# LayoutLLM-T2I/LayoutLLM-T2I

Hardware: AMD Instinct MI355X
Metric: 512x512 50-step images/sec (PLMS, CFG 7.5, layout-conditioned GLIGEN UNet) (higher is better)
Workload: dtype fp16 (fp32 accumulate); 1 GPU; configs[1]: 512x512, 50 PLMS steps, batch=4/GPU, 8 grounding boxes/image, fp16; survey_config=2, unet_forwards_per_image=102, parallelism=replicas x1, one weight broadcast, no per-step collectives

## Files before the change

layoutllm_t2i_amd/csrc/gemm8.hip:

```cpp
#include "common.h"
#include "gligen_hip.h"
#include "gemm_shared.h"
#include "opts.h"
#include <atomic>
#include <type_traits>

#ifndef G8_S3_PHASES
#define G8_S3_PHASES 3
#endif

namespace {

template <int BM_, int BN>
struct G8 {
    static constexpr int BM = BM_;
    static constexpr int NA = BM / 64;
    static constexpr int MI = BM / 64;
    static constexpr int MH = BM / 128;
    static constexpr int BK = 64;
    static constexpr int PW = BN / 2;
    static constexpr int TN = PW / 16;
    static constexpr int A_BYTES = BM * BK * 2;
    static constexpr int B_BYTES = BN * BK * 2;
    static constexpr int STAGE = A_BYTES + B_BYTES;
// ... 306 lines not shown
            }
        };
        constexpr int XA = 5;
        const half_t* xptr[XA];
        unsigned xrb = 0u;
#pragma unroll
        for (int u = 0; u < XA; ++u) {
            const int j = 8 * (u < 4 ? 4 * wave + u : 32) + srow;
            const int mc = m0 - 1 + j;
            xptr[u] = zsrc;
            if (mc >= 0 && mc < M) {
                int oy, ox;
                pix(mc, oy, ox);
                xrb |= ((oy >= 1 ? 1u : 0u) | 2u | (oy + 1 < cg.Hin ? 4u : 0u)) << (3 * u);
                xptr[u] = cg.in + (size_t)mc * cg.Cin + ((sslot ^ ((j >> 1) & 7)) << 3);
            }
        }
        const int xrow = 64 * wm + lr;
        auto xfrag = [&](const int j) __attribute__((always_inline)) -> int { return j * 128 + ((lq ^ ((j >> 1) & 7)) << 4); };
        const int xzero = X::A_BYTES + (lq << 4);
        const int xo1 = xfrag(xrow + 1);
        int xo0[MI], xo2[MI];
#pragma unroll
        for (int mi = 0; mi < MI; ++mi) {
            int oy, ox;
            pix(m0 + xrow + 16 * mi, oy, ox);
            xo0[mi] = ox == 0 ? xzero : xfrag(xrow + 16 * mi);
            xo2[mi] = ox == cg.Win - 1 ? xzero : xfrag(xrow + 16 * mi + 2);
        }
        const int xb_off = (PW * grp + lr) * 128 + fsw;
        if (tid < 16) *reinterpret_cast<uint4*>(smem + (tid >> 3) * X::A_STRIDE + X::A_BYTES + ((tid & 7) << 4)) = make_uint4(0u, 0u, 0u, 0u);
        asm volatile("s_waitcnt lgkmcnt(0)" ::: "memory");

        int xa_ky = 0, xa_cb = kt_begin / 9, xb_kt = kt_begin;
        int xa_off = -cg.Win * cg.Cin + (xa_cb << 6);
        int xa_rd = 0, xa_is = 0, xb_rd = 0, xb_is = 0;
        auto xa_advance = [&]() __attribute__((always_inline)) {
            if (++xa_ky == 3) { xa_ky = 0; ++xa_cb; }
            xa_off = (xa_ky - 1) * cg.Win * cg.Cin + (xa_cb << 6);
        };
        auto x_src = [&](const int id) __attribute__((always_inline)) -> const half_t* {
            const half_t* src;
            if (id < 8) {
                const uint64_t a = reinterpret_cast<uint64_t>(xptr[id < XA ? id : 0] + xa_off), z = reinterpret_cast<uint64_t>(zsrc);
                const uint64_t keep = (uint64_t)0 - (uint64_t)((xrb >> (3 * id + xa_ky)) & 1u);
                src = reinterpret_cast<const half_t*>((a & keep) | (z & ~keep));
                if constexpr (DBG & 2) src = zsrc;
            } else {
                const int j = id - 8 < C::NB0 ? id - 8 : 0;
                src = ((bmask >> j) & 1u) ? bptr[j] + (xb_kt << 6) : zsrc;
                if constexpr (DBG & 4) src = zsrc;
            }
            return src;
        };
        auto x_fire = [&](const int id, const half_t* src) __attribute__((always_inline)) {
            if (id < 8) glds16(src, reinterpret_cast<half_t*>(smem + xa_is * X::A_STRIDE + (id < 4 ? 4 * wave + id : 32) * 1024));
            else glds16(src, reinterpret_cast<half_t*>(smem + X::B_BASE + xb_is * X::B_BYTES + (bunit0 + id - 8) * 1024));
        };
        const bool has_a4 = wave == 4;
        const bool has_b2 = C::NB0 > 2 && nb > 2;

#pragma unroll
        for (int u = 0; u < 4; ++u) x_fire(u, x_src(u));
        if (has_a4) x_fire(4, x_src(4));
        xa_advance();
        xa_is = 1;
#pragma unroll
        for (int s = 0; s < 2; ++s) {
// ... 237 lines not shown
    } else {
        for (; t + 2 < nkt; ++t) ktile(std::true_type{});
        for (; t < nkt; ++t) ktile(std::false_type{});
    }
    if (grp == 0) G8_SBAR();
    if constexpr (DBG & 1) ts2 = __builtin_readcyclecounter();

    constexpr int EPS = PW + 4;
    constexpr int CG8 = PW / 8;
    constexpr int ITEMS = 32 * CG8;
    static_assert(ITEMS % 64 == 0, "whole sweeps");
    float* stage = reinterpret_cast<float*>(smem) + wave * (32 * EPS);
    const int epi = p.epi;
    const float* __restrict__ bias = p.bias;
    float gate = 1.0f;
    if (splitk == 1 && epi == GL_EPI_GATE_RES) gate = p.gate[0];
    const int nbase = n0 + PW * grp;
    half_t* outp = reinterpret_cast<half_t*>(p.out);
    constexpr int NQ = ITEMS / 64;
    const bool vt_wave = p.vt != nullptr && nbase >= p.vt_col0;
    const bool generic = splitk == 1 && !vt_wave && epi != GL_EPI_GEGLU;
    auto orow = [&](const int m) __attribute__((always_inline)) -> int {
        if constexpr (UPF) {
            const int hw = cg.Hin * cg.Win;
            const int b = m / hw;
            const int rr = m - b * hw;
            const int y = rr / cg.Win;
            const int x = rr - y * cg.Win;
            return (b * cg.Hout + 2 * y + py) * cg.Wout + 2 * x + px;
        } else {
            return m;
        }
    };
    Fin8Aux aux[MH][NQ];
    if (generic) {
#pragma unroll
        for (int h = 0; h < MH; ++h)
#pragma unroll
            for (int q = 0; q < NQ; ++q) {
                const int idx = lane + 64 * q;
                const int r = idx / CG8, c = (idx - r * CG8) * 8;
                const int m = m0 + (BM / 4) * wm + 32 * h + r, n = nbase + c;
                if (m < Mrows && n < N) fin8_load(p, orow(m), n, aux[h][q]);
            }
    }
    float vt_bias[2] = {0.0f, 0.0f};
    if (splitk == 1 && vt_wave && bias) {
#pragma unroll
        for (int j = 0; j < 2; ++j) {
            const int col = 64 * j + lane;
            if (col < PW && nbase + col < N) vt_bias[j] = bias[nbase + col];
        }
    }
    float gg_bias[16];
#pragma unroll
    for (int j = 0; j < 16; ++j) gg_bias[j] = 0.0f;
    if constexpr (PW == 64) {
        if (splitk == 1 && epi == GL_EPI_GEGLU && bias) {
            const int nx = nbase + (lane & 3) * 8;
            if (nx < N) {
#pragma unroll
                for (int j = 0; j < 8; ++j) { gg_bias[j] = bias[nx + j]; gg_bias[8 + j] = bias[nx + 32 + j]; }
            }
        }
    }
#pragma unroll
// ... 82 lines not shown
                        const float4 g0 = *reinterpret_cast<const float4*>(stage + r * EPS + pc + 32);
                        const float4 g1 = *reinterpret_cast<const float4*>(stage + r * EPS + pc + 36);
                        float xv[8] = {x0.x, x0.y, x0.z, x0.w, x1.x, x1.y, x1.z, x1.w};
                        float gv[8] = {g0.x, g0.y, g0.z, g0.w, g1.x, g1.y, g1.z, g1.w};
                        half8_t o, lo8 = {};
#pragma unroll
                        for (int j = 0; j < 8; ++j) {
                            const float a = xv[j] + gg_bias[j], b = gv[j] + gg_bias[8 + j];
                            float y = a * gelu_erf_f(b);
                            if (p.out_mode == GL_OUT_F16_HILO) y = pin_value(y);
                            o[j] = (half_t)y;
                            if (p.out_mode == GL_OUT_F16_HILO) lo8[j] = (half_t)(y - (float)o[j]);
                        }
                        st16(outp + (size_t)m * p.ldc + (nbase >> 1) + pc, *reinterpret_cast<uint4*>(&o));
                        if (p.out_mode == GL_OUT_F16_HILO) st16(outp + (size_t)m * p.ldc + (N >> 1) + (nbase >> 1) + pc, *reinterpret_cast<uint4*>(&lo8));
                    }
                }
            }
        } else {
#pragma unroll
            for (int q = 0; q < NQ; ++q) {
                const int idx = lane + 64 * q;
                const int r = idx / CG8, c = (idx - r * CG8) * 8;
                const int m = mbase + r, n = nbase + c;
                if (m < Mrows && n < N) {
                    const float4 a0 = *reinterpret_cast<const float4*>(stage + r * EPS + c);
                    const float4 a1 = *reinterpret_cast<const float4*>(stage + r * EPS + c + 4);
                    float v[8] = {a0.x, a0.y, a0.z, a0.w, a1.x, a1.y, a1.z, a1.w};
                    fin8_store(p, gate, orow(m), n, v, aux[h][q]);
                }
            }
        }
    }
    if constexpr (DBG & 1) {
        asm volatile("s_waitcnt vmcnt(0)" ::: "memory");
        const unsigned long long ts3 = __builtin_readcyclecounter();
        const int bid = blockIdx.x + gridDim.x * blockIdx.z;
        if (tid == 0 && bid < 4096) {
            g8_stamps[4 * bid + 0] = ts0; g8_stamps[4 * bid + 1] = ts1; g8_stamps[4 * bid + 2] = ts2; g8_stamps[4 * bid + 3] = ts3;
        }
    }
}

#define g8_dbg gl_opt(32)
#define g8_kxr gl_opt(54)

std::atomic<uint64_t> g8_kxr_launches{0};
std::atomic<uint64_t> g8_upf_launches{0};

static bool kxr_default(const gl_gemm_args&, const ConvGeom&, int , int ) { return true; }

constexpr int G8_MAX_DEVICES = 64;
const half_t* g8_zero_page[G8_MAX_DEVICES] = {};

template <int BM, int BN, bool CONV, bool S3 = false>
int launch8(const gl_gemm_args& g, const ConvGeom& cg_in, int zs, int kper, int order_m, hipStream_t st) {
    int dev = -1;
    if (hipGetDevice(&dev) != hipSuccess || dev < 0 || dev >= G8_MAX_DEVICES) return GL_ERR_BAD_ARG;
    if (!g8_zero_page[dev]) return GL_ERR_BAD_ARG;
    ConvGeom cg = cg_in;
    cg.zero = g8_zero_page[dev];
    const int mt = gl_cdiv(g.M, BM), nt = gl_cdiv(g.N, BN);
    dim3 grid(mt * nt, 1, zs);
    bool done = false;
    if (cg.ups == 2) {
        if constexpr (CONV && !S3) {
            grid.x = 4 * gl_cdiv(cg.B * cg.Hin * cg.Win, BM) * nt;
            gemm8_kernel<BM, BN, true, 0, false, false, true><<<grid, dim3(512), G8<BM, BN>::LDS, st>>>(g, cg, zs, kper, order_m);
            GL_CHECK_LAUNCH();
            g8_upf_launches.fetch_add(1, std::memory_order_relaxed);
            return 0;
        } else {
            return GL_ERR_UNSUPPORTED;
        }
    }
    if constexpr (CONV && !S3 && BM == 256) {
        const bool eligible = cg.stride == 1 && !cg.ups && cg.shift == 0 && g.kwrap == 0 && cg.cwrap == 0 && !(order_m & 2) && kper > 0 &&
                              (kper % 9) == 0 && cg.Hin == cg.Hout && cg.Win == cg.Wout && g.K == 9 * cg.Cin && g.a2 == nullptr;
        if (eligible && (g8_kxr == 1 || (g8_kxr == 2 && kxr_default(g, cg, BN, zs)))) {
            void (*k)(gl_gemm_args, ConvGeom, int, int, int) = gemm8_kernel<BM, BN, true, 0, false, true>;
            if constexpr (BN == 160) {
                if (g8_dbg == 1) k = gemm8_kernel<BM, BN, true, 1, false, true>;
                if (g8_dbg == 3) k = gemm8_kernel<BM, BN, true, 3, false, true>;
            }
            k<<<grid, dim3(512), G8X<BN>::LDS, st>>>(g, cg, zs, kper, order_m);
            GL_CHECK_LAUNCH();
            g8_kxr_launches.fetch_add(1, std::memory_order_relaxed);
            return 0;
        }
    }
    if constexpr (S3) {
        gemm8_kernel<BM, BN, CONV, 0, true><<<grid, dim3(512), G8<BM, BN>::LDS, st>>>(g, cg, zs, kper, order_m);
        done = true;
    } else if constexpr (BN == 160 && BM == 256) {
        void (*k)(gl_gemm_args, ConvGeom, int, int, int) = nullptr;
        if (g8_dbg == 1) k = gemm8_kernel<BM, BN, CONV, 1>;
        if (g8_dbg == 3) k = gemm8_kernel<BM, BN, CONV, 3>;
        if (k) {
            k<<<grid, dim3(512), G8<BM, BN>::LDS, st>>>(g, cg, zs, kper, order_m);
            done = true;
        }
    }
    if (!done) gemm8_kernel<BM, BN, CONV><<<grid, dim3(512), G8<BM, BN>::LDS, st>>>(g, cg, zs, kper, order_m);
    GL_CHECK_LAUNCH();
    return 0;
}

template <int BM, int BN, bool CONV>
int set_attr8() {
    hipError_t e = hipFuncSetAttribute((const void*)gemm8_kernel<BM, BN, CONV>, hipFuncAttributeMaxDynamicSharedMemorySize, G8<BM, BN>::LDS);
    if (e == hipSuccess) e = hipFuncSetAttribute((const void*)gemm8_kernel<BM, BN, CONV, 0, true>, hipFuncAttributeMaxDynamicSharedMemorySize, G8<BM, BN>::LDS);
    if constexpr (CONV) {
// ... 31 lines not shown

template <bool S3>
static int gl8_launch_t(const gl_gemm_args& g, const ConvGeom& cg, bool conv, int bm, int bn, int zs, int kper, int order_m, hipStream_t st) {
    if (bm == 256 && bn == 160) return conv ? launch8<256, 160, true, S3>(g, cg, zs, kper, order_m, st) : launch8<256, 160, false, S3>(g, cg, zs, kper, order_m, st);
    if (bm == 256 && bn == 128) return conv ? launch8<256, 128, true, S3>(g, cg, zs, kper, order_m, st) : launch8<256, 128, false, S3>(g, cg, zs, kper, order_m, st);
    if (bm == 128 && bn == 160) return conv ? launch8<128, 160, true, S3>(g, cg, zs, kper, order_m, st) : launch8<128, 160, false, S3>(g, cg, zs, kper, order_m, st);
    if (bm == 128 && bn == 128) return conv ? launch8<128, 128, true, S3>(g, cg, zs, kper, order_m, st) : launch8<128, 128, false, S3>(g, cg, zs, kper, order_m, st);
    return GL_ERR_UNSUPPORTED;
}
int gl8_launch(const gl_gemm_args& g, const ConvGeom& cg, bool conv, int bm, int bn, int zs, int kper, int order_m, hipStream_t st, bool s3) {
    return s3 ? gl8_launch_t<true>(g, cg, conv, bm, bn, zs, kper, order_m, st) : gl8_launch_t<false>(g, cg, conv, bm, bn, zs, kper, order_m, st);
}

int gl8_init(void) {
    int e;
    void* zp = nullptr;
    int dev = -1;
    if (hipGetDevice(&dev) != hipSuccess || dev < 0 || dev >= G8_MAX_DEVICES) return GL_ERR_BAD_ARG;
    if (hipGetSymbolAddress(&zp, HIP_SYMBOL(g_zero16)) != hipSuccess) return GL_ERR_BAD_ARG;
    g8_zero_page[dev] = reinterpret_cast<const half_t*>(zp);
    if ((e = set_attr8<256, 160, false>())) return e;
    if ((e = set_attr8<256, 160, true>())) return e;
    if ((e = set_attr8<256, 128, false>())) return e;
    if ((e = set_attr8<256, 128, true>())) return e;
    if ((e = set_attr8<128, 160, false>())) return e;
    if ((e = set_attr8<128, 160, true>())) return e;
    if ((e = set_attr8<128, 128, false>())) return e;
    if ((e = set_attr8<128, 128, true>())) return e;
    return 0;
}

uint64_t gl8_kxr_launch_count(void) { return g8_kxr_launches.load(std::memory_order_relaxed); }
uint64_t gl8_upf_launch_count(void) { return g8_upf_launches.load(std::memory_order_relaxed); }

int gl8_read_stamps(void* dst, int64_t bytes) {
    if (bytes > (int64_t)sizeof(unsigned long long) * 4 * 4096) return GL_ERR_BAD_ARG;
    hipError_t e = hipMemcpyFromSymbol(dst, HIP_SYMBOL(g8_stamps), (size_t)bytes, 0, hipMemcpyDeviceToHost);
    void* p = nullptr;
    if (e == hipSuccess) e = hipGetSymbolAddress(&p, HIP_SYMBOL(g8_stamps));
    if (e == hipSuccess) e = hipMemset(p, 0, sizeof(unsigned long long) * 4 * 4096);
    return (int)e;
}
```

layoutllm_t2i_amd/csrc/gemm_conv.hip:

```cpp
#include <atomic>
#include <cstring>
#include "common.h"
#include "gligen_hip.h"
#include "gemm_shared.h"
#include "opts.h"

namespace {

#define g_opt_ksplit gl_opt(13)
#define g_opt_geglu32 gl_opt(8)
#define g_opt_big gl_opt(7)
#define g_opt_small gl_opt(4)
#define g_opt_splitk_tiles gl_opt(5)
#define g_opt_splitk_tiles_conv gl_opt(GL_OPT_SPLITK_TILES_CONV)
#define g_opt_splitk_nk gl_opt(6)
#define g_opt_skinny gl_opt(24)
#define g_opt_order gl_opt(23)
#define g_opt_tile gl_opt(2)
#define g_opt_g8 gl_opt(30)
#define g_opt_g8_tiles gl_opt(31)
#define g_opt_g8_tapmajor gl_opt(33)
#define g_opt_g8_minkt gl_opt(34)
std::atomic<uint64_t> g8_launches{0};
#define g_opt_g8_shortk gl_opt(37)
#define g_opt_g8_bm128 gl_opt(46)
#define g_opt_g8_minblk gl_opt(47)
#define g_opt_g8_s3 gl_opt(52)
#define g_opt_g8_minnk gl_opt(35)

template <int BM, int BN, int BKT, int NW = 4>
constexpr int lds_bytes() {
    constexpr int pipe = 2 * (BM + BN) * BKT * (int)sizeof(half_t);
    constexpr int epi = NW * 32 * 68 * (int)sizeof(float);
    return pipe > epi ? pipe : epi;
}

template <int BM, int BN, int BKT, int WK = 1>
constexpr int min_waves() {
    if (WK > 1) return 2;
    if (BKT != 32) return 1;
    if (BM * BN >= 256 * 128) return 2;
    if (BM * BN <= 128 * 128) return 4;
    return 3;
}

template <int BM, int BN, int WAVES_M, int WAVES_N, bool CONV, int BKT, int WK = 1>
__global__ __launch_bounds__(64 * WAVES_M * WAVES_N * WK, (min_waves<BM, BN, BKT, WK>())) void gemm_kernel(gl_gemm_args p, ConvGeom cg, int splitk, int kt_per_split, int order_m) {
    constexpr int NTHR = 64 * WAVES_M * WAVES_N * WK;
    constexpr int TM = BM / WAVES_M / 32;
    constexpr int TN = BN / WAVES_N / 32;
    constexpr int CPR = BKT / 8;
    constexpr int RPP = NTHR / CPR;
    constexpr int RPW = 64 / CPR;
    constexpr int APASS = (BM + RPP - 1) / RPP;
    constexpr int BPASS = (BN + RPP - 1) / RPP;
    constexpr int KSTEPS = BKT / 16;
    static_assert(WAVES_M * WAVES_N * WK == 4, "4 waves");
    static_assert(WK == 1 || (WK == 2 && TM == 2 && KSTEPS % 2 == 0), "K-split: two groups, two 32-row tiles per wave");
    static_assert(BM % RPW == 0 && BN % RPW == 0, "whole wave instructions");
    static_assert(BKT == 64 || BKT == 32, "BK");
// ... 610 lines not shown
                            g.vt_ld < g.vt_rows || g.vt_H * g.vt_d != g.N - g.vt_col0))
        return GL_ERR_BAD_ARG;
    if constexpr (!CONV) {
        if (g.vt_lo == nullptr && skinny_ok(g)) {
            gemm_skinny_kernel<<<dim3(g.N / 32, gl_cdiv(g.M, 32)), dim3(256), 0, st>>>(g);
            GL_CHECK_LAUNCH();
            return 0;
        }
    }
    const bool need8 = g.vt_lo != nullptr;
    if (need8) {
        int bn_ = 0;
        if (!g_opt_g8 || !gl8_supported(g, CONV, &bn_)) return GL_ERR_UNSUPPORTED;
    }
    const bool upf = CONV && cg.ups == 2;
    auto mtiles = [&](const int bm_) { return upf ? 4 * gl_cdiv(g.M / 4, bm_) : gl_cdiv(g.M, bm_); };
    if (g_opt_g8 || upf) {
        int bn = 0;
        if (gl8_supported(g, CONV, &bn, upf)) {
            const int nk = g.K / 64;
            auto plan_split = [&](const int tiles_) {
                int sk = 1;
                if (tiles_ < g_opt_g8_tiles && g.workspace && g.epi != GL_EPI_GEGLU && g.vt == nullptr) {
                    sk = 256 / tiles_;
                    if (sk > nk / g_opt_g8_minkt) sk = nk / g_opt_g8_minkt;
                    while (sk > 1 && (int64_t)sk * g.M * g.N * 4 > g.workspace_bytes) --sk;
                    if (sk < 1) sk = 1;
                }
                return sk;
            };
            int bm = 256;
            int tiles = mtiles(256) * gl_cdiv(g.N, bn);
            int splitk = plan_split(tiles);
            if (tiles * 2 <= 256 && g.epi != GL_EPI_GEGLU && g.vt == nullptr) {
                const bool want = CONV ? ((g_opt_g8_bm128 & 4) || ((g_opt_g8_bm128 & 1) && nk / splitk <= 16)) : ((g_opt_g8_bm128 & 2) != 0);
                if (want) {
                    bm = 128;
                    tiles = mtiles(128) * gl_cdiv(g.N, bn);
                    splitk = plan_split(tiles);
                }
            }
            if (!CONV && (g_opt_g8_bm128 & 8) && bm == 256 && splitk == 1 && tiles > 256 && g.epi != GL_EPI_GEGLU) {
                const int t128 = gl_cdiv(g.M, 128) * gl_cdiv(g.N, bn);
                auto fills = [](const int b) { return b * 5 >= ((b + 255) / 256) * 256 * 4; };
                if (!fills(tiles) && fills(t128) && t128 <= 2048) {
                    bm = 128;
                    tiles = t128;
                }
            }
            if (!CONV && splitk > 1 && nk / splitk < 20) splitk = nk / 20 > 0 ? nk / 20 : 1;
            bool enough = tiles * splitk >= (CONV ? g_opt_g8_tiles : (g_opt_g8_minblk < g_opt_g8_tiles ? g_opt_g8_minblk : g_opt_g8_tiles)) && nk >= g_opt_g8_minnk;
            if (!CONV && enough) {
                const int blocks = tiles * splitk;
                const bool full_rounds = g_opt_g8_shortk && blocks * 5 >= ((blocks + 255) / 256) * 256 * 4;
                enough = nk >= 16 || blocks <= 256 || (g.epi == GL_EPI_GEGLU && (nk >= 10 || full_rounds)) || (full_rounds && blocks <= 2048);
            }
            if (g_opt_g8 == 2 || enough || need8 || upf) {
                const bool s3 = g_opt_g8_s3 != 0 && g.kwrap != 0 && g.K == 3 * g.kwrap &&
                                (CONV ? cg.cwrap != 0 : (g.a2 == g.a && g.lda2 == g.lda && g.ksplit == 2 * g.kwrap));
                const int nks = s3 ? g.kwrap / 32 : nk;
                const int kper = gl_cdiv(nks, splitk);
                const int zs = gl_cdiv(nks, kper);
                const int order_m = g_opt_order == 1 ? ((CONV ? 9L : 1L) * g.N > (long)g.M) : (g_opt_order == 2);
                const int e = gl8_launch(g, cg, CONV, bm, bn, zs, kper, order_m | (CONV && g_opt_g8_tapmajor ? 2 : 0), st, s3);
                if (e) return e;
                if (!upf) g8_launches.fetch_add(1, std::memory_order_relaxed);
                if (zs > 1) {
                    const size_t total = (size_t)g.M * (g.N / 8);
                    int nblk = (int)((total + 255) / 256);
                    if (nblk > 2048) nblk = 2048;
                    splitk_reduce_kernel<<<dim3(nblk), dim3(256), 0, st>>>(g, zs);
                    GL_CHECK_LAUNCH();
                }
                return 0;
            }
        }
    }
    if (upf) return GL_ERR_UNSUPPORTED;
    if constexpr (!CONV) {
        if (g_opt_geglu32 && g.epi == GL_EPI_GEGLU && g.K <= 640 && g.a2 == nullptr) return dispatch_shape<false, 32>(g, cg, st);
    }
    return dispatch_shape<CONV, 64>(g, cg, st);
}

}

extern "C" int gl_gemm(const gl_gemm_args* a, void* stream) {
    if (!a || !a->a || !a->w || !a->out) return GL_ERR_BAD_ARG;
    ConvGeom cg{};
    gl_gemm_args g = *a;
    if (g.kwrap != 0 && ((g.kwrap % 64) != 0 || g.kwrap >= g.K || g.K > 3 * g.kwrap)) return GL_ERR_BAD_ARG;
    if (g.ldw == 0) g.ldw = g.kwrap != 0 ? g.kwrap : g.K;
    if (g.ldw < (g.kwrap != 0 ? (g.K > 2 * g.kwrap ? 2 * g.kwrap : g.kwrap) : g.K) || (g.ldw % 8) != 0) return GL_ERR_BAD_ARG;
    return dispatch<false>(g, cg, (hipStream_t)stream);
// ... 39 lines not shown
int set_lds_attr() {
    hipError_t e = hipFuncSetAttribute((const void*)gemm_kernel<BM, BN, WM, WN, CONV, BKT, WK>,
                                       hipFuncAttributeMaxDynamicSharedMemorySize, lds_bytes<BM, BN, BKT, WM * WN * WK>());
    return e == hipSuccess ? 0 : (int)e;
}
template <int BM, int BN, int WM, int WN, int BKT, int WK = 1>
int set_lds_attr2() {
    int e = set_lds_attr<BM, BN, WM, WN, false, BKT, WK>();
    return e ? e : set_lds_attr<BM, BN, WM, WN, true, BKT, WK>();
}

extern "C" int gl_init_gemm(void) {
    int e;
    if ((e = set_lds_attr2<64, 128, 2, 2, 64>())) return e;
    if ((e = set_lds_attr2<128, 128, 2, 2, 64>())) return e;
    if ((e = set_lds_attr2<128, 160, 4, 1, 64>())) return e;
    if ((e = set_lds_attr2<256, 64, 4, 1, 64>())) return e;
    if ((e = set_lds_attr2<128, 160, 2, 1, 64, 2>())) return e;
    if ((e = set_lds_attr2<128, 128, 2, 1, 64, 2>())) return e;
    if ((e = set_lds_attr<64, 128, 1, 2, false, 64, 2>())) return e;
    if ((e = set_lds_attr2<256, 160, 4, 1, 32>())) return e;
    if ((e = set_lds_attr2<256, 128, 4, 1, 32>())) return e;
    if ((e = set_lds_attr<64, 128, 2, 2, false, 32>())) return e;
    if ((e = set_lds_attr<128, 128, 2, 2, false, 32>())) return e;
    if ((e = gl8_init())) return e;
    return 0;
}

int gl_attn_read_launch_counts(void* dst, int64_t bytes);

extern "C" int gl_debug_read(int what, void* dst, int64_t bytes) {
    if (what == 8) return gl8_read_stamps(dst, bytes);
    if (what == 10) return gl_attn_read_launch_counts(dst, bytes);
    if (what == 9 || what == 11 || what == 12) {
        if (!dst || bytes < (int64_t)sizeof(uint64_t)) return GL_ERR_BAD_ARG;
        const uint64_t n = what == 9 ? g8_launches.load(std::memory_order_relaxed) : (what == 11 ? gl8_kxr_launch_count() : gl8_upf_launch_count());
        memcpy(dst, &n, sizeof n);
        return 0;
    }
    return GL_ERR_BAD_ARG;
}
```

layoutllm_t2i_amd/csrc/gemm_shared.h:

```cpp
#pragma once
#include "common.h"
#include "gligen_hip.h"

static __device__ uint4 g_zero16[4];

struct ConvGeom {
    const half_t* in;
    int B, Hin, Win, Cin, Hout, Wout, stride, ups;
    const half_t* zero;
    int cwrap;
    int shift;
};

namespace {

__device__ __forceinline__ void wait_vmcnt0() { asm volatile("s_waitcnt vmcnt(0)" ::: "memory"); }

__device__ __forceinline__ void glds16(const half_t* src, half_t* dst) {
    __builtin_amdgcn_global_load_lds(
        reinterpret_cast<const __attribute__((address_space(1))) void*>(reinterpret_cast<uintptr_t>(src)),
        reinterpret_cast<__attribute__((address_space(3))) void*>(reinterpret_cast<uintptr_t>(dst)), 16, 0, 0);
}

struct Fin8Aux {
// ... 64 lines not shown
        ld16o = p.ldc2;
        if (o16 == nullptr) return;
    }
    if (p.out_mode == GL_OUT_F16_HILO) {
#pragma unroll
        for (int j = 0; j < 8; ++j) v[j] = pin_value(v[j]);
    }
    half8_t o;
#pragma unroll
    for (int j = 0; j < 8; ++j) o[j] = (half_t)v[j];
    st16(o16 + (size_t)m * ld16o + n, *reinterpret_cast<uint4*>(&o));
    if (p.out_mode == GL_OUT_F16_HILO) {
        half8_t l;
#pragma unroll
        for (int j = 0; j < 8; ++j) l[j] = (half_t)(v[j] - (float)o[j]);
        st16(o16 + (size_t)m * ld16o + p.N + n, *reinterpret_cast<uint4*>(&l));
    }
}

__device__ __forceinline__ void finish8(const gl_gemm_args& p, float gate, int m, int n, float (&v)[8]) {
    Fin8Aux a;
    fin8_load(p, m, n, a);
    fin8_store(p, gate, m, n, v, a);
}

}

int gl8_supported(const gl_gemm_args& g, bool conv, int* bn_out, bool upfold = false);
int gl8_launch(const gl_gemm_args& g, const ConvGeom& cg, bool conv, int bm, int bn, int zs, int kper, int order_m, hipStream_t st, bool s3 = false);
int gl8_init(void);
int gl8_read_stamps(void* dst, int64_t bytes);
uint64_t gl8_kxr_launch_count(void);
uint64_t gl8_upf_launch_count(void);
```

layoutllm_t2i_amd/csrc/misc.hip:

```cpp
#include "common.h"
#include "gligen_hip.h"
#include "opts.h"

#include <initializer_list>

namespace {

template <typename OT>
__global__ __launch_bounds__(256) void posnet_input_kernel(const float* __restrict__ boxes, const float* __restrict__ masks,
                                                           const float* __restrict__ emb, const float* __restrict__ null_pos,
                                                           const float* __restrict__ null_xyxy, int in_dim, int num_freqs,
                                                           OT* __restrict__ out) {
    const int row = blockIdx.x;
    const float m = masks[row];
    const int pos_dim = num_freqs * 8;
    OT* o = out + (size_t)row * (in_dim + pos_dim);
    for (int c = threadIdx.x; c < in_dim; c += 256) {
        const float v = emb[(size_t)row * in_dim + c] * m + (1.0f - m) * null_pos[c];
        o[c] = (OT)v;
    }
    for (int c = threadIdx.x; c < pos_dim; c += 256) {
        const int j = c / 8;
        const int r = c - j * 8;
        const int coord = r & 3;
// ... 653 lines not shown

extern "C" int gl_latent_affine_pack(const float* z, const float* w, const float* bias, float pre, int32_t B, int32_t C,
                                     int32_t hw, int32_t Cpad, void* out, void* stream) {
    if (!z || !w || !bias || !out || B <= 0 || C <= 0 || hw <= 0 || Cpad < C) return GL_ERR_BAD_ARG;
    latent_affine_pack_kernel<<<dim3(ew_blocks((size_t)B * hw * Cpad)), dim3(256), 0, (hipStream_t)stream>>>(
        z, w, bias, pre, B, C, hw, Cpad, reinterpret_cast<half_t*>(out));
    GL_CHECK_LAUNCH();
    return 0;
}

extern "C" int gl_init_gemm(void);
extern "C" int gl_init_ff(void);
extern "C" int gl_init_attn(void);
static gl_opts make_default_opts() {
    gl_opts o{};
    o.v[2] = 0;    o.v[3] = 0;    o.v[4] = 400;  o.v[5] = 300;  o.v[GL_OPT_SPLITK_TILES_CONV] = 450;
    o.v[6] = 16;   o.v[7] = 300;  o.v[8] = 1;    o.v[10] = -1;  o.v[13] = 3;
    o.v[16] = 16;  o.v[17] = 1;   o.v[20] = 0;   o.v[21] = 1;   o.v[23] = 1;
    o.v[24] = 64;  o.v[25] = 1;   o.v[27] = 1;   o.v[29] = 1;   o.v[30] = 1;
    o.v[31] = 200; o.v[32] = 0;   o.v[33] = 0;   o.v[34] = 11;  o.v[35] = 5;
    o.v[37] = 1;
    o.v[41] = 1;
    o.v[42] = 1;
    o.v[43] = 1;
    o.v[38] = 1;
    o.v[44] = 1;
    o.v[45] = 1024;
    o.v[46] = 11;
    o.v[47] = 100;
    o.v[50] = 0;
    o.v[51] = 1;
    o.v[52] = 1;
    o.v[55] = 2;
    o.v[54] = 2;
    return o;
}
gl_opts g_gl_opts = make_default_opts();
thread_local const gl_opts* tl_gl_opts = nullptr;
int g_gl_option_epoch = 0;

bool gl_opts_put(gl_opts& t, int key, int value) {
    switch (key) {
        case 2: case 3: case 4: case 6: case 7: case 8: case 10: case 13: case 17: case 20: case 21: case 23: case 24: case 25:
        case 27: case 29: case 30: case 31: case 32: case 33: case 35: case 37: case 38: case 41: case 42: case 43: case 44: case 45: case 46: case 47: case 50: case 51: case 52: case 53: case 54: case 55:
            t.v[key] = value;
            return true;
        case 5:
            t.v[5] = value < 0 ? 300 : value;
            t.v[GL_OPT_SPLITK_TILES_CONV] = value < 0 ? 450 : value;
            return true;
        case 16: t.v[16] = value > 0 ? value : 16; return true;
        case 34: t.v[34] = value < 1 ? 1 : value; return true;
        default: return false;
    }
}

extern "C" int gl_get_option(int key) {
    if (key < 0 || key >= GL_OPT_MAX) return GL_ERR_BAD_ARG;
    return g_gl_opts.v[key];
}

extern "C" int gl_set_option(int key, int value) {
    if (key < 0 || key >= GL_OPT_MAX || !gl_opts_put(g_gl_opts, key, value)) return GL_ERR_BAD_ARG;
    ++g_gl_option_epoch;
    return 0;
}

extern "C" int gl_abi_version(void) { return GL_ABI_VERSION; }
extern "C" int gl_sizeof_gemm_args(void) { return (int)sizeof(gl_gemm_args); }
extern "C" int gl_sizeof_conv_args(void) { return (int)sizeof(gl_conv_args); }
extern "C" int gl_sizeof_attn_args(void) { return (int)sizeof(gl_attn_args); }
extern "C" int gl_sizeof_gn_args(void) { return (int)sizeof(gl_gn_args); }
extern "C" int gl_init(void) {
    int e = gl_init_gemm();
    if (!e) e = gl_init_ff();
    return e ? e : gl_init_attn();
}
```

layoutllm_t2i_amd/csrc/opts.h:

```cpp
#pragma once
#include <cstdint>

constexpr int GL_OPT_MAX = 56;
constexpr int GL_OPT_SPLITK_TILES_CONV = 40;

struct gl_opts {
    int v[GL_OPT_MAX];
};

struct gl_opt_overrides {
    uint64_t mask = 0;
    int v[GL_OPT_MAX] = {};
    int epoch = 0;
};

extern gl_opts g_gl_opts;
extern int g_gl_option_epoch;
extern thread_local const gl_opts* tl_gl_opts;

static inline int gl_opt(int key) {
    const gl_opts* o = tl_gl_opts;
    return (o ? o : &g_gl_opts)->v[key];
}

bool gl_opts_put(gl_opts& t, int key, int value);

struct gl_opts_scope {
    gl_opts eff;
    const gl_opts* prev;
    explicit gl_opts_scope(const gl_opt_overrides& o) : prev(tl_gl_opts) {
        eff = g_gl_opts;
        for (int k = 0; k < GL_OPT_MAX; ++k)
            if ((o.mask >> k) & 1u) gl_opts_put(eff, k, o.v[k]);
        tl_gl_opts = &eff;
    }
    ~gl_opts_scope() { tl_gl_opts = prev; }
// ... 4 lines not shown
```

layoutllm_t2i_amd/ops.py:

```python
from __future__ import annotations

import ctypes as C
from typing import Optional

import torch

from . import _lib
from ._lib import (EPI_BIAS, EPI_GATE_RES, EPI_GEGLU, EPI_RES, EPI_ROWBIAS, EPI_SILU, OUT_F16_HILO, OUT_F16_ROWMAJOR, OUT_F32_NCHW,
                   OUT_F32_ROWMAJOR, AttnArgs, ConvArgs, GemmArgs, GnArgs, check)

F16 = torch.float16
F32 = torch.float32


_DEV = None


def _stream() -> int:
    dev = _DEV if _DEV is not None else torch.cuda.current_device()
    if dev != torch.cuda.current_device():
        raise _lib.HipLibraryError(f"tensors live on cuda:{dev} but cuda:{torch.cuda.current_device()} is current: wrap the "
                                   "call in torch.cuda.device(...) (kernels launch on the current device)")
    _lib.init_device(dev)
    return torch.cuda.current_stream(dev).cuda_stream
# ... 628 lines not shown
        _req(t, F32, n, 4)
    _req(out, F16, "out")
    B, Cc, h, ww = z.shape
    check(_lib.lib().gl_latent_affine_pack(z.data_ptr(), w.data_ptr(), bias.data_ptr(), pre, B, Cc, h * ww, Cpad,
                                           out.data_ptr(), _stream()), "gl_latent_affine_pack")
    return out


def set_option(key: int, value: int) -> None:
    check(_lib.lib().gl_set_option(key, value), "gl_set_option")


def gemm8_launch_count() -> int:
    import ctypes
    n = ctypes.c_uint64(0)
    check(_lib.lib().gl_debug_read(9, ctypes.byref(n), 8), "gl_debug_read")
    return int(n.value)


def kxreuse_launch_count() -> int:
    import ctypes
    n = ctypes.c_uint64(0)
    check(_lib.lib().gl_debug_read(11, ctypes.byref(n), 8), "gl_debug_read")
    return int(n.value)


def upfold_launch_count() -> int:
    import ctypes
    n = ctypes.c_uint64(0)
    check(_lib.lib().gl_debug_read(12, ctypes.byref(n), 8), "gl_debug_read")
    return int(n.value)


ATTN_FORMS = ("split_pipe", "split_8w", "split_4w_dbuf", "split_4w_single", "f16_8w_pre0", "f16_8w_pre1", "f16_8w_pre2", "f16_4w_pre0",
              "f16_4w_pre1", "f16_4w_pre2")


def attention_launch_counts() -> dict:
    import ctypes
    n = (ctypes.c_uint64 * len(ATTN_FORMS))()
    check(_lib.lib().gl_debug_read(10, ctypes.byref(n), ctypes.sizeof(n)), "gl_debug_read")
    return {k: int(v) for k, v in zip(ATTN_FORMS, n)}


def clip_patchify(pixel_values: torch.Tensor, patch: int, Kpad: int, out: torch.Tensor) -> torch.Tensor:
    _req(pixel_values, F32, "pixel_values")
    _req(out, F16, "out")
    B, c3, S, S2 = pixel_values.shape
    if c3 != 3 or S != S2 or not pixel_values.is_contiguous():
        raise ValueError("pixel_values must be a contiguous [B, 3, S, S] tensor")
    check(_lib.lib().gl_clip_patchify(pixel_values.data_ptr(), B, S, patch, Kpad, out.data_ptr(), _stream()), "gl_clip_patchify")
    return out


def clip_assemble(patch_emb: torch.Tensor, class_emb: torch.Tensor, pos_emb: torch.Tensor, B: int, T: int, x: torch.Tensor,
                  ln_gamma: Optional[torch.Tensor] = None, ln_beta: Optional[torch.Tensor] = None, eps: float = 1e-5) -> torch.Tensor:
    _req(patch_emb, F16, "patch_emb")
    for t, n in ((class_emb, "class_emb"), (pos_emb, "pos_emb"), (x, "x")):
        _req(t, F32, n)
    C_ = x.shape[-1]
    check(_lib.lib().gl_clip_assemble(patch_emb.data_ptr(), _rows(patch_emb, "patch_emb")[2], class_emb.data_ptr(), pos_emb.data_ptr(), B, T, C_,
                                      _ptr(ln_gamma), _ptr(ln_beta), eps, x.data_ptr(), _stream()), "gl_clip_assemble")
    return x


def clip_embed_tokens(ids: torch.Tensor, tok_emb: torch.Tensor, pos_emb: torch.Tensor, x: torch.Tensor) -> torch.Tensor:
# ... 228 lines not shown
```

Before: 4.988 images/s.

## Allow row-aligned k-split for reuse conv kernel and direct split-K partial stores

Conv split-K slices may now begin mid-tap-group: the reuse kernel computes the starting kernel row from kt_begin, and a planner picks a split size that is a multiple of three while fitting the grid and workspace. A new direct split-K epilogue writes fp32 partial accumulators straight from registers to the workspace, skipping the LDS staging path. Both are enabled by default (opt 54=3, opt 56=1). This lets more split-K conv launches use the kx-reuse kernel and shortens the partial-write epilogue. The trade-off is uncoalesced float4 stores and extra option plumbing.

Result: no change. 5.002 images/s, median of 6 (+0.3%).

```diff
diff --git a/layoutllm_t2i_amd/csrc/gemm8.hip b/layoutllm_t2i_amd/csrc/gemm8.hip
--- a/layoutllm_t2i_amd/csrc/gemm8.hip
+++ b/layoutllm_t2i_amd/csrc/gemm8.hip
@@ -362,8 +362,9 @@
         if (tid < 16) *reinterpret_cast<uint4*>(smem + (tid >> 3) * X::A_STRIDE + X::A_BYTES + ((tid & 7) << 4)) = make_uint4(0u, 0u, 0u, 0u);
         asm volatile("s_waitcnt lgkmcnt(0)" ::: "memory");
 
-        int xa_ky = 0, xa_cb = kt_begin / 9, xb_kt = kt_begin;
-        int xa_off = -cg.Win * cg.Cin + (xa_cb << 6);
+        int xa_cb = kt_begin / 9, xb_kt = kt_begin;
+        int xa_ky = (kt_begin - 9 * xa_cb) / 3;
+        int xa_off = (xa_ky - 1) * cg.Win * cg.Cin + (xa_cb << 6);
         int xa_rd = 0, xa_is = 0, xb_rd = 0, xb_is = 0;
         auto xa_advance = [&]() __attribute__((always_inline)) {
             if (++xa_ky == 3) { xa_ky = 0; ++xa_cb; }
@@ -667,6 +668,32 @@
             return m;
         }
     };
+    auto write_stamps = [&]() __attribute__((always_inline)) {
+        if constexpr (DBG & 1) {
+            asm volatile("s_waitcnt vmcnt(0)" ::: "memory");
+            const unsigned long long ts3 = __builtin_readcyclecounter();
+            const int bid = blockIdx.x + gridDim.x * blockIdx.z;
+            if (tid == 0 && bid < 4096) {
+                g8_stamps[4 * bid + 0] = ts0; g8_stamps[4 * bid + 1] = ts1; g8_stamps[4 * bid + 2] = ts2; g8_stamps[4 * bid + 3] = ts3;
+            }
+        }
+    };
+    if (splitk > 1 && (order_flags & 4)) {
+        float* ws = reinterpret_cast<float*>(p.workspace) + (size_t)blockIdx.z * M * N + nbase + 4 * lq;
+#pragma unroll
+        for (int mi = 0; mi < MI; ++mi) {
+            const int m = m0 + (BM / 4) * wm + 16 * mi + lr;
+            if (m < Mrows) {
+                float* o = ws + (size_t)orow(m) * N;
+#pragma unroll
+                for (int ni = 0; ni < TN; ++ni)
+                    if (nbase + 16 * ni + 4 * lq < N)
+                        *reinterpret_cast<float4*>(o + 16 * ni) = make_float4(acc[mi][ni][0], acc[mi][ni][1], acc[mi][ni][2], acc[mi][ni][3]);
+            }
+        }
+        write_stamps();
+        return;
+    }
     Fin8Aux aux[MH][NQ];
     if (generic) {
 #pragma unroll
@@ -815,21 +842,17 @@
             }
         }
     }
-    if constexpr (DBG & 1) {
-        asm volatile("s_waitcnt vmcnt(0)" ::: "memory");
-        const unsigned long long ts3 = __builtin_readcyclecounter();
-        const int bid = blockIdx.x + gridDim.x * blockIdx.z;
-        if (tid == 0 && bid < 4096) {
-            g8_stamps[4 * bid + 0] = ts0; g8_stamps[4 * bid + 1] = ts1; g8_stamps[4 * bid + 2] = ts2; g8_stamps[4 * bid + 3] = ts3;
-        }
-    }
+    write_stamps();
 }
 
 #define g8_dbg gl_opt(32)
 #define g8_kxr gl_opt(54)
+#define g8_direct gl_opt(56)
 
 std::atomic<uint64_t> g8_kxr_launches{0};
 std::atomic<uint64_t> g8_upf_launches{0};
+std::atomic<uint64_t> g8_splitk_launches{0};
+std::atomic<uint64_t> g8_splitk_direct_launches{0};
 
 static bool kxr_default(const gl_gemm_args&, const ConvGeom&, int , int ) { return true; }
 
@@ -837,12 +860,15 @@
 const half_t* g8_zero_page[G8_MAX_DEVICES] = {};
 
 template <int BM, int BN, bool CONV, bool S3 = false>
-int launch8(const gl_gemm_args& g, const ConvGeom& cg_in, int zs, int kper, int order_m, hipStream_t st) {
+int launch8(const gl_gemm_args& g, const ConvGeom& cg_in, int zs, int kper, int order_in, hipStream_t st) {
+    const int order_m = order_in | (zs > 1 && g8_direct ? 4 : 0);
     int dev = -1;
     if (hipGetDevice(&dev) != hipSuccess || dev < 0 || dev >= G8_MAX_DEVICES) return GL_ERR_BAD_ARG;
     if (!g8_zero_page[dev]) return GL_ERR_BAD_ARG;
     ConvGeom cg = cg_in;
     cg.zero = g8_zero_page[dev];
+    if (zs > 1) g8_splitk_launches.fetch_add(1, std::memory_order_relaxed);
+    if (order_m & 4) g8_splitk_direct_launches.fetch_add(1, std::memory_order_relaxed);
     const int mt = gl_cdiv(g.M, BM), nt = gl_cdiv(g.N, BN);
     dim3 grid(mt * nt, 1, zs);
     bool done = false;
@@ -859,8 +885,9 @@
     }
     if constexpr (CONV && !S3 && BM == 256) {
         const bool eligible = cg.stride == 1 && !cg.ups && cg.shift == 0 && g.kwrap == 0 && cg.cwrap == 0 && !(order_m & 2) && kper > 0 &&
-                              (kper % 9) == 0 && cg.Hin == cg.Hout && cg.Win == cg.Wout && g.K == 9 * cg.Cin && g.a2 == nullptr;
-        if (eligible && (g8_kxr == 1 || (g8_kxr == 2 && kxr_default(g, cg, BN, zs)))) {
+                              ((kper % 9) == 0 || (g8_kxr >= 3 && (kper % 3) == 0)) && cg.Hin == cg.Hout && cg.Win == cg.Wout && g.K == 9 * cg.Cin &&
+                              g.a2 == nullptr;
+        if (eligible && (g8_kxr == 1 || (g8_kxr >= 2 && kxr_default(g, cg, BN, zs)))) {
             void (*k)(gl_gemm_args, ConvGeom, int, int, int) = gemm8_kernel<BM, BN, true, 0, false, true>;
             if constexpr (BN == 160) {
                 if (g8_dbg == 1) k = gemm8_kernel<BM, BN, true, 1, false, true>;
@@ -958,6 +985,10 @@
 
 uint64_t gl8_kxr_launch_count(void) { return g8_kxr_launches.load(std::memory_order_relaxed); }
 uint64_t gl8_upf_launch_count(void) { return g8_upf_launches.load(std::memory_order_relaxed); }
+void gl8_splitk_launch_counts(uint64_t out[2]) {
+    out[0] = g8_splitk_launches.load(std::memory_order_relaxed);
+    out[1] = g8_splitk_direct_launches.load(std::memory_order_relaxed);
+}
 
 int gl8_read_stamps(void* dst, int64_t bytes) {
     if (bytes > (int64_t)sizeof(unsigned long long) * 4 * 4096) return GL_ERR_BAD_ARG;
diff --git a/layoutllm_t2i_amd/csrc/gemm_conv.hip b/layoutllm_t2i_amd/csrc/gemm_conv.hip
--- a/layoutllm_t2i_amd/csrc/gemm_conv.hip
+++ b/layoutllm_t2i_amd/csrc/gemm_conv.hip
@@ -26,6 +26,7 @@
 #define g_opt_g8_bm128 gl_opt(46)
 #define g_opt_g8_minblk gl_opt(47)
 #define g_opt_g8_s3 gl_opt(52)
+#define g_opt_g8_gemm_minkt gl_opt(57)
 #define g_opt_g8_minnk gl_opt(35)
 
 template <int BM, int BN, int BKT, int NW = 4>
@@ -702,7 +703,16 @@
             int bm = 256;
             int tiles = mtiles(256) * gl_cdiv(g.N, bn);
             int splitk = plan_split(tiles);
-            if (tiles * 2 <= 256 && g.epi != GL_EPI_GEGLU && g.vt == nullptr) {
+            int kya_kper = 0;
+            if constexpr (CONV) {
+                if (gl_opt(54) >= 3 && splitk > 1 && cg.stride == 1 && !cg.ups && cg.shift == 0 && g.kwrap == 0 && cg.cwrap == 0 && !g_opt_g8_tapmajor &&
+                    cg.Hin == cg.Hout && cg.Win == cg.Wout && g.K == 9 * cg.Cin) {
+                    int kp = (g_opt_g8_minkt + 2) / 3 * 3;
+                    while (kp < nk && ((int64_t)gl_cdiv(nk, kp) * tiles > 256 || (int64_t)gl_cdiv(nk, kp) * g.M * g.N * 4 > g.workspace_bytes)) kp += 3;
+                    if (kp < nk) kya_kper = kp;
+                }
+            }
+            if (tiles * 2 <= 256 && g.epi != GL_EPI_GEGLU && g.vt == nullptr && !(kya_kper && gl_opt(54) >= 4)) {
                 const bool want = CONV ? ((g_opt_g8_bm128 & 4) || ((g_opt_g8_bm128 & 1) && nk / splitk <= 16)) : ((g_opt_g8_bm128 & 2) != 0);
                 if (want) {
                     bm = 128;
@@ -710,6 +720,8 @@
                     splitk = plan_split(tiles);
                 }
             }
+            if (bm != 256) kya_kper = 0;
+            if (kya_kper) splitk = gl_cdiv(nk, kya_kper);
             if (!CONV && (g_opt_g8_bm128 & 8) && bm == 256 && splitk == 1 && tiles > 256 && g.epi != GL_EPI_GEGLU) {
                 const int t128 = gl_cdiv(g.M, 128) * gl_cdiv(g.N, bn);
                 auto fills = [](const int b) { return b * 5 >= ((b + 255) / 256) * 256 * 4; };
@@ -718,7 +730,7 @@
                     tiles = t128;
                 }
             }
-            if (!CONV && splitk > 1 && nk / splitk < 20) splitk = nk / 20 > 0 ? nk / 20 : 1;
+            if (!CONV && splitk > 1 && nk / splitk < g_opt_g8_gemm_minkt) splitk = nk / g_opt_g8_gemm_minkt > 0 ? nk / g_opt_g8_gemm_minkt : 1;
             bool enough = tiles * splitk >= (CONV ? g_opt_g8_tiles : (g_opt_g8_minblk < g_opt_g8_tiles ? g_opt_g8_minblk : g_opt_g8_tiles)) && nk >= g_opt_g8_minnk;
             if (!CONV && enough) {
                 const int blocks = tiles * splitk;
@@ -729,7 +741,7 @@
                 const bool s3 = g_opt_g8_s3 != 0 && g.kwrap != 0 && g.K == 3 * g.kwrap &&
                                 (CONV ? cg.cwrap != 0 : (g.a2 == g.a && g.lda2 == g.lda && g.ksplit == 2 * g.kwrap));
                 const int nks = s3 ? g.kwrap / 32 : nk;
-                const int kper = gl_cdiv(nks, splitk);
+                const int kper = kya_kper ? kya_kper : gl_cdiv(nks, splitk);
                 const int zs = gl_cdiv(nks, kper);
                 const int order_m = g_opt_order == 1 ? ((CONV ? 9L : 1L) * g.N > (long)g.M) : (g_opt_order == 2);
                 const int e = gl8_launch(g, cg, CONV, bm, bn, zs, kper, order_m | (CONV && g_opt_g8_tapmajor ? 2 : 0), st, s3);
@@ -835,6 +847,13 @@
 extern "C" int gl_debug_read(int what, void* dst, int64_t bytes) {
     if (what == 8) return gl8_read_stamps(dst, bytes);
     if (what == 10) return gl_attn_read_launch_counts(dst, bytes);
+    if (what == 13) {
+        uint64_t n[2];
+        if (!dst || bytes < (int64_t)sizeof n) return GL_ERR_BAD_ARG;
+        gl8_splitk_launch_counts(n);
+        memcpy(dst, n, sizeof n);
+        return 0;
+    }
     if (what == 9 || what == 11 || what == 12) {
         if (!dst || bytes < (int64_t)sizeof(uint64_t)) return GL_ERR_BAD_ARG;
         const uint64_t n = what == 9 ? g8_launches.load(std::memory_order_relaxed) : (what == 11 ? gl8_kxr_launch_count() : gl8_upf_launch_count());
diff --git a/layoutllm_t2i_amd/csrc/gemm_shared.h b/layoutllm_t2i_amd/csrc/gemm_shared.h
--- a/layoutllm_t2i_amd/csrc/gemm_shared.h
+++ b/layoutllm_t2i_amd/csrc/gemm_shared.h
@@ -120,3 +120,4 @@
 int gl8_read_stamps(void* dst, int64_t bytes);
 uint64_t gl8_kxr_launch_count(void);
 uint64_t gl8_upf_launch_count(void);
+void gl8_splitk_launch_counts(uint64_t out[2]);
diff --git a/layoutllm_t2i_amd/csrc/misc.hip b/layoutllm_t2i_amd/csrc/misc.hip
--- a/layoutllm_t2i_amd/csrc/misc.hip
+++ b/layoutllm_t2i_amd/csrc/misc.hip
@@ -709,7 +709,9 @@
     o.v[51] = 1;
     o.v[52] = 1;
     o.v[55] = 2;
-    o.v[54] = 2;
+    o.v[54] = 3;
+    o.v[57] = 20;
+    o.v[56] = 1;
     return o;
 }
 gl_opts g_gl_opts = make_default_opts();
@@ -719,7 +721,7 @@
 bool gl_opts_put(gl_opts& t, int key, int value) {
     switch (key) {
         case 2: case 3: case 4: case 6: case 7: case 8: case 10: case 13: case 17: case 20: case 21: case 23: case 24: case 25:
-        case 27: case 29: case 30: case 31: case 32: case 33: case 35: case 37: case 38: case 41: case 42: case 43: case 44: case 45: case 46: case 47: case 50: case 51: case 52: case 53: case 54: case 55:
+        case 27: case 29: case 30: case 31: case 32: case 33: case 35: case 37: case 38: case 41: case 42: case 43: case 44: case 45: case 46: case 47: case 50: case 51: case 52: case 53: case 54: case 55: case 56:
             t.v[key] = value;
             return true;
         case 5:
@@ -728,6 +730,7 @@
             return true;
         case 16: t.v[16] = value > 0 ? value : 16; return true;
         case 34: t.v[34] = value < 1 ? 1 : value; return true;
+        case 57: t.v[57] = value < 1 ? 1 : value; return true;
         default: return false;
     }
 }
diff --git a/layoutllm_t2i_amd/csrc/opts.h b/layoutllm_t2i_amd/csrc/opts.h
--- a/layoutllm_t2i_amd/csrc/opts.h
+++ b/layoutllm_t2i_amd/csrc/opts.h
@@ -1,7 +1,7 @@
 #pragma once
 #include <cstdint>
 
-constexpr int GL_OPT_MAX = 56;
+constexpr int GL_OPT_MAX = 58;
 constexpr int GL_OPT_SPLITK_TILES_CONV = 40;
 
 struct gl_opts {
diff --git a/layoutllm_t2i_amd/ops.py b/layoutllm_t2i_amd/ops.py
--- a/layoutllm_t2i_amd/ops.py
+++ b/layoutllm_t2i_amd/ops.py
@@ -684,6 +684,13 @@
     return int(n.value)
 
 
+def splitk8_launch_counts() -> tuple:
+    import ctypes
+    n = (ctypes.c_uint64 * 2)()
+    check(_lib.lib().gl_debug_read(13, ctypes.byref(n), ctypes.sizeof(n)), "gl_debug_read")
+    return int(n[0]), int(n[1])
+
+
 ATTN_FORMS = ("split_pipe", "split_8w", "split_4w_dbuf", "split_4w_single", "f16_8w_pre0", "f16_8w_pre1", "f16_8w_pre2", "f16_4w_pre0",
               "f16_4w_pre1", "f16_4w_pre2")
 
```
